# HIITMetagenomics/dsm-framework

Hardware: AMD Instinct MI355X
Metric: enumerated substrings/sec (Emax=2.0) (higher is better)
Workload: dtype u32

## Files before the change

dsm-framework_amd/csrc/emit_runs.h:

```cpp
#pragma once
#include <algorithm>
#include <cstdint>
#include <cstring>
#include <vector>

namespace dsm {

inline void kept_runs(const uint8_t* keep, uint32_t nt, uint8_t drop, std::vector<uint32_t>& seg) {
    seg.clear();
    uint32_t from = 0;
    for (const uint8_t* q = keep; (q = (const uint8_t*)memchr(q, drop, (size_t)(keep + nt - q))) != nullptr; ++q) {
        const uint32_t r = (uint32_t)(q - keep);
        if (r > from) { seg.push_back(from); seg.push_back(r); }
        from = r + 1;
    }
    if (nt > from) { seg.push_back(from); seg.push_back(nt); }
}

inline void rebase_runs(uint32_t* rel_path, uint32_t* rel_pair, const std::vector<uint32_t>& seg, const std::vector<uint32_t>& bp,
                        const std::vector<uint32_t>& bq, uint32_t lo, uint32_t hi) {
    const size_t ns = seg.size() / 2;
    size_t i = (size_t)(std::upper_bound(seg.begin(), seg.end(), lo) - seg.begin()) / 2;
    if (i > 0 && lo <= seg[2 * (i - 1) + 1]) --i;
    for (; i < ns && seg[2 * i] < hi; ++i) {
        const uint32_t a = seg[2 * i] > lo ? seg[2 * i] : lo, b = seg[2 * i + 1] + 1 < hi ? seg[2 * i + 1] + 1 : hi;
        const uint32_t sp = bp[i], sq = bq[i];
        if (!sp && !sq) continue;
        for (uint32_t r = a; r < b; ++r) { rel_path[r] -= sp; rel_pair[r] -= sq; }
    }
}

}
```

dsm-framework_amd/csrc/engine.hip:

```cpp
#include <sched.h>

#include <algorithm>
#include <atomic>
#include <chrono>
#include <cmath>
#include <condition_variable>
#include <cstdlib>
#include <cstring>
#include <deque>
#include <map>
#include <functional>
#include <memory>
#include <mutex>
#include <sstream>
#include <thread>
#include <type_traits>

#include "common.h"
#include "scan.h"
#include "setorder.h"
#include "stream_parse.h"
#include "lfstep.h"
#include "entropy_tables.h"
#include "textemit.h"
#include "engine_api.h"
#include "emit_runs.h"

namespace dsm {

__device__ __forceinline__ u64 wave_sum_u64(u64 v) {
#pragma unroll
    for (int d = 32; d >= 1; d >>= 1) v += __shfl_xor(v, d, 64);
    return v;
}


struct Kids {
    const u64* plane;
    const u32* cum;
};
__device__ __forceinline__ u32 kid_mask(const Kids& k, u32 v) {
    const u64* p = k.plane + (size_t)(v >> 6) * 4;
    const u32 s = v & 63;
    return (u32)((p[0] >> s) & 1) | ((u32)((p[1] >> s) & 1) << 1) | ((u32)((p[2] >> s) & 1) << 2) | ((u32)((p[3] >> s) & 1) << 3);
}
__device__ __forceinline__ u32 kid_index(const Kids& k, u32 v, u32 c) {
    const size_t e = (size_t)(v >> 6) * 4 + c;
    return k.cum[e] + (u32)__popcll(k.plane[e] & ((1ull << (v & 63)) - 1));
}
// ... 1 lines not shown
struct KidWave {
    u64 p[4];
    u32 c[4];
};
__device__ __forceinline__ void kid_wave(const Kids& k, u32 w, KidWave& o) {
#pragma unroll
    for (int c = 0; c < 4; ++c) { o.p[c] = k.plane[(size_t)w * 4 + c]; o.c[c] = k.cum[(size_t)w * 4 + c]; }
}
__device__ __forceinline__ u32 bits_below_lane(u64 p) {
    return __builtin_amdgcn_mbcnt_hi((u32)(p >> 32), __builtin_amdgcn_mbcnt_lo((u32)p, 0u));
}

constexpr u32 NUM_XCD = 8;
__device__ __forceinline__ u32 xcd_block() {
    const u32 b = blockIdx.x, G = gridDim.x;
    const u32 x = b % NUM_XCD, i = b / NUM_XCD, per = G / NUM_XCD, rem = G % NUM_XCD;
    return x * per + (x < rem ? x : rem) + i;
}

constexpr int NPT = 4;
static inline dim3 grid_npt(u64 n) { return dim3((unsigned)((n + 256ull * NPT - 1) / (256ull * NPT))); }


static inline void timeline(const char* what, const char* arg = "") {
    static const bool on = getenv("DSM_TIMELINE") != nullptr;
    if (!on) return;
    static const auto t0 = std::chrono::steady_clock::now();
    fprintf(stderr, "dsm timeline %9.3f ms  %s %s\n", std::chrono::duration<double, std::milli>(std::chrono::steady_clock::now() - t0).count(), what, arg);
}

constexpr u32 BC_OK = 0x4f4b4f4bu, BC_CAPACITY = 0x46554c4cu, BC_ABORT = 0x41424f52u;
constexpr u32 XHDR = 16;
struct ExpandChain {
    struct Link { hipEvent_t last = nullptr; const void* owner = nullptr; };
    std::mutex mu;
    std::map<int, Link> dev;
};
static ExpandChain g_expand_chain;

struct Xchg {
    const u8* base;
    u64 bpr;
    u32 nlocal;
    u32 d;
    u64 F;
    u32 fb;
    u32 nm;
};
__device__ __forceinline__ u64 x_word_index(const Xchg& x, u32 l, u64 v) { return x.nm ? v * x.nlocal + l : (u64)l * x.F + v; }
// ... 918 lines not shown
    u32 r = start[v] + sub[v] - 1;
    slot[r] = RankSlot{k, level};
    if (npair) npair[r] = crec ? 1u : (k + 1 < ncand ? cand_poff[k + 1] : npairs) - cand_poff[k];
}

struct LevelDev {
    const uint2* pw;
    const u32* cand_node;
    const u32* cand_poff;
    const uint4* crec;
    const u32* ids;
    const u64* freqs;
};

constexpr int EMIT_MAX_CHUNKS = 8;
struct ChunkBounds { u32 tb[EMIT_MAX_CHUNKS + 1]; int n; };
__global__ void chunk_bounds_kernel(ChunkBounds cbs, const u32* __restrict__ path_off, const u32* __restrict__ pair_off, u32* __restrict__ out) {
    const int c = threadIdx.x;
    if (c <= cbs.n) { out[2 * c] = path_off[cbs.tb[c]]; out[2 * c + 1] = pair_off ? pair_off[cbs.tb[c]] : cbs.tb[c]; }
}

constexpr u8 EV_DROP = 0, EV_KEEP = 1, EV_HOST = 2;
struct FillVerdict {
    double* ent;
    u8* keep;
    u32* rel_path;
    u32* rel_pair;
    u32* counts;
    const double* terms;
    const double* logn;
    const u32* bounds;
    u32 chunk, d;
    double emin, emax;
};
__global__ __launch_bounds__(256) void tuple_fill_kernel(u32 nlev, const LevelDev* __restrict__ lv, const u32* __restrict__ path_off,
                                                         const u32* __restrict__ pair_off, const RankSlot* __restrict__ slot, char* __restrict__ paths,
                                                         u32* __restrict__ ids, u64* __restrict__ freqs, u32 rank_lo, u32 rank_hi, FillVerdict fv) {
    constexpr u32 LDS_LEVELS = 1024;
    __shared__ const uint2* s_pw[LDS_LEVELS];
    __shared__ u32 s_text[256];
    const u32 nl = nlev < LDS_LEVELS ? nlev : LDS_LEVELS;
    for (u32 q = threadIdx.x; q < nl; q += blockDim.x) s_pw[q] = lv[q].pw;
    {
        const u32 b = threadIdx.x;
        s_text[b] = ((0x54474341u >> (8 * (b & 3))) & 0xFFu) | (((0x54474341u >> (8 * ((b >> 2) & 3))) & 0xFFu) << 8) |
                    (((0x54474341u >> (8 * ((b >> 4) & 3))) & 0xFFu) << 16) | (((0x54474341u >> (8 * ((b >> 6) & 3))) & 0xFFu) << 24);
    }
    __syncthreads();
    const u32 r = rank_lo + blockIdx.x * blockDim.x + threadIdx.x;
    if (r >= rank_hi) return;
    const u32 p_first = path_off[r], p_end = path_off[r + 1];
    const u32 o_first = pair_off ? pair_off[r] : r, o_end = pair_off ? pair_off[r + 1] : r + 1;
    const u32 lvl = p_end - p_first;
    const u32 k = slot[r].k;
    const LevelDev L = lv[lvl];
    const bool one = L.crec != nullptr;
    const uint4 cr = one ? L.crec[k] : make_uint4(0u, 0u, 0u, 0u);
    const u32 b = one ? k : L.cand_poff[k];
    u64 sumN = fv.d;
    double sl = 0;
    bool beyond = false;
    for (u32 q = b, o = o_first; o < o_end; ++q, ++o) {
        const u64 fq = one ? (((u64)cr.w << 32) | cr.z) : L.freqs[q];
        if (ids) ids[o] = one ? 0u : L.ids[q];
        freqs[o] = fq;
        sumN += fq;
        if (fv.ent && !beyond) {
            if (fq < TERM_TAB) sl += fv.terms[fq]; else beyond = true;
        }
    }
    if (fv.ent) {
        beyond = beyond || sumN >= LOGN_TAB;
        u8 verdict = EV_HOST;
        if (!beyond) {
            const double en = fv.logn[sumN] - sl / (double)sumN;
            fv.ent[r] = en;
            verdict = (fv.emax > 0 && (en < fv.emin || en > fv.emax)) ? EV_DROP : EV_KEEP;
        }
        const u32 pb0 = fv.bounds[2 * fv.chunk], qb0 = fv.bounds[2 * fv.chunk + 1];
        fv.keep[r] = verdict;
        fv.rel_path[r + fv.chunk] = p_first - pb0;
        fv.rel_pair[r + fv.chunk] = o_first - qb0;
        if (r + 1 == rank_hi) {
            fv.rel_path[r + 1 + fv.chunk] = p_end - pb0;
            fv.rel_pair[r + 1 + fv.chunk] = o_end - qb0;
        }
        const u64 md = __ballot(verdict == EV_DROP), mh = __ballot(verdict == EV_HOST);
        if ((md | mh) && (threadIdx.x & 63) == (u32)(__ffsll((long long)__ballot(1)) - 1)) {
            if (md) atomicAdd(fv.counts, (u32)__popcll(md));
            if (mh) atomicAdd(fv.counts + 1, (u32)__popcll(mh));
        }
    }
    u32 v = one ? cr.x : L.cand_node[k];
    char* dst = paths + p_first;
    u32 l = lvl;
    while (l > 0) {
        const u32 first = ((l - 1) / PW_CHUNK) * PW_CHUNK;
        const uint2 w = (l < LDS_LEVELS ? s_pw[l] : lv[l].pw)[v];
        const u32 cnt = l - first;
        const u32 q0 = s_text[w.y & 0xFFu], q1 = s_text[(w.y >> 8) & 0xFFu], q2 = s_text[(w.y >> 16) & 0xFFu], q3 = s_text[w.y >> 24];
        char* d = dst + first;
        if (cnt == PW_CHUNK) {
            __builtin_memcpy(d, &q0, 4); __builtin_memcpy(d + 4, &q1, 4); __builtin_memcpy(d + 8, &q2, 4); __builtin_memcpy(d + 12, &q3, 4);
        } else {
            const u32 full = cnt >> 2;
            if (full > 0) __builtin_memcpy(d, &q0, 4);
            if (full > 1) __builtin_memcpy(d + 4, &q1, 4);
            if (full > 2) __builtin_memcpy(d + 8, &q2, 4);
// ... 264 lines not shown
        if (e != hipSuccess) return fail(DSM_E_NOMEM, std::string("hipHostMalloc: ") + hipGetErrorString(e));
        cap = want;
        return 0;
    }
    ~PinBuf() { if (p) (void)hipHostFree(p); }
};
struct DevGrow {
    void* p = nullptr;
    size_t cap = 0;
    int ensure(size_t n) {
        if (n <= cap) return 0;
        if (p) (void)hipFree(p);
        p = nullptr;
        cap = 0;
        size_t want = n + n / 4 + 4096;
        hipError_t e = hipMalloc(&p, want);
        if (e != hipSuccess) return fail(DSM_E_NOMEM, std::string("hipMalloc: ") + hipGetErrorString(e));
        cap = want;
        return 0;
    }
    ~DevGrow() { if (p) (void)hipFree(p); }
};
struct EmitSet {
    DevGrow dev[10];
    hipEvent_t ready = nullptr;
    static constexpr int MAX_CHUNKS = EMIT_MAX_CHUNKS;
    int nchunk = 1;
    u32 cb[MAX_CHUNKS + 1] = {0};
    hipEvent_t cready[MAX_CHUNKS] = {nullptr};
    int device = 0;
    PinBuf pin[10];
    u64 pb[MAX_CHUNKS + 1] = {0}, qb[MAX_CHUNKS + 1] = {0};
    RawBuf out[6];
    u32 nt = 0;
    bool busy = false;
    ~EmitSet() {
        if (ready) (void)hipEventDestroy(ready);
        for (auto e : cready) if (e) (void)hipEventDestroy(e);
    }
};

struct HostPool {
    std::vector<std::thread> th;
    std::mutex mu;
    std::condition_variable cv, done_cv;
    std::function<void(unsigned)> job;
    unsigned gen = 0, pending = 0;
    bool stop = false;
    void ensure(unsigned n) {
        while (th.size() + 1 < n) {
            const unsigned id = (unsigned)th.size() + 1;
            th.emplace_back([this, id] {
                unsigned seen = 0;
                for (;;) {
// ... 18 lines not shown
    unsigned active = 0;
    void run(unsigned n, const std::function<void(unsigned)>& f) {
        ensure(n);
        {
            std::lock_guard<std::mutex> lk(mu);
            job = f; active = n; pending = n - 1; ++gen;
        }
        cv.notify_all();
        f(0u);
        std::unique_lock<std::mutex> lk(mu);
        done_cv.wait(lk, [&] { return pending == 0; });
    }
    ~HostPool() {
        {
            std::lock_guard<std::mutex> lk(mu);
            stop = true;
        }
        cv.notify_all();
        for (auto& t : th) t.join();
    }
};

static int emit_job(HostPool& pool, EmitSet& E, int c, u32 d, double emin, double emax, dsm_tuple_sink sink, void* ctx, std::vector<u32>& zero_ids,
                    u64* n_tuples, u64* n_pairs, double* ms) {
    struct timespec t0, t1;
    clock_gettime(CLOCK_MONOTONIC, &t0);
    const u32 t_lo = E.cb[c], t_hi = E.cb[c + 1];
    const u32 nt = t_hi - t_lo;
    u32* rel_path = (u32*)E.pin[0].p + t_lo + c;
    u32* rel_pair = (u32*)E.pin[1].p + t_lo + c;
    u32* ids = (u32*)E.pin[2].p + E.qb[c];
    if (d == 1) {
        const size_t need = (size_t)rel_pair[nt] + 1;
        if (zero_ids.size() < need) zero_ids.resize(need + need / 4, 0u);
        ids = zero_ids.data();
    }
    u64* freqs = (u64*)E.pin[3].p + E.qb[c];
    char* paths = (char*)E.pin[4].p + E.pb[c];
    double* ent = (double*)E.pin[5].p + t_lo;
    u8* keep = (u8*)E.pin[6].p + t_lo;
    const u32* counts = (const u32*)E.pin[9].p + 2 * c;
    u64 ndrop = counts[0];
    if (counts[1]) {
        for (u8* q = keep; (q = (u8*)memchr(q, EV_HOST, (size_t)(keep + nt - q))) != nullptr; ++q) {
            const u32 r = (u32)(q - keep);
            const double e = exact_entropy(d, freqs + rel_pair[r], rel_pair[r + 1] - rel_pair[r]);
            ent[r] = e;
            const bool k = !(emax > 0 && (e < emin || e > emax));
            keep[r] = k ? EV_KEEP : EV_DROP;
            if (!k) ++ndrop;
        }
    }
    static const bool tl_on = getenv("DSM_TIMELINE") != nullptr;
    if (tl_on) { char msg[96]; snprintf(msg, sizeof msg, "nt=%u dropped=%llu host=%u", nt, (unsigned long long)ndrop, counts[1]); timeline("  emitter: verdicts", msg); }
    u64 W = nt, QW = rel_pair[nt];
    u32* o_path = rel_path;
    u32* o_pair = rel_pair;
    double* o_ent = ent;
    char* o_paths = paths;
    u32* o_ids = ids;
    u64* o_freqs = freqs;
    constexpr u64 FEW_DROPS = 4096;
    if (ndrop && ndrop <= FEW_DROPS && ndrop * 64 < nt) {
        std::vector<u32> seg;
        kept_runs(keep, nt, EV_DROP, seg);
        const size_t ns = seg.size() / 2;
        std::vector<u32> bp(ns), bq(ns);
        for (size_t i = 0; i < ns; ++i) { bp[i] = rel_path[seg[2 * i]]; bq[i] = rel_pair[seg[2 * i]]; }
        unsigned nth = host_threads();
        if (nt < 65536) nth = 1;
        const u32 per = (nt + nth - 1) / nth;
        auto rebase = [&](unsigned t) {
            const u32 lo = t * per < nt ? t * per : nt, hi = t + 1 == nth ? nt + 1 : (lo + per < nt ? lo + per : nt);
            rebase_runs(rel_path, rel_pair, seg, bp, bq, lo, hi);
        };
        pool.run(nth, rebase);
        clock_gettime(CLOCK_MONOTONIC, &t1);
        *ms += (t1.tv_sec - t0.tv_sec) * 1e3 + (t1.tv_nsec - t0.tv_nsec) * 1e-6;
        for (size_t i = 0; i < ns; ++i) {
            const u32 a = seg[2 * i], n = seg[2 * i + 1] - a;
            *n_tuples += n;
            *n_pairs += rel_pair[a + n];
            if (!sink) continue;
            dsm_tuple_batch bt;
            bt.ntuples = n;
            bt.path_off = rel_path + a; bt.path_bytes = paths + bp[i]; bt.entropy = ent + a;
            bt.pair_off = rel_pair + a; bt.ids = ids + bq[i]; bt.freqs = freqs + bq[i];
            if (sink(ctx, &bt)) return 1;
        }
        return 0;
    }
    if (ndrop) {
        unsigned nth = host_threads();
        if (nt < 65536) nth = 1;
        const u32 per = (nt + nth - 1) / nth;
        std::vector<u64> cnt_t(nth + 1, 0), cnt_p(nth + 1, 0), cnt_q(nth + 1, 0);
        auto range = [&](unsigned t, u32& lo, u32& hi) { lo = t * per < nt ? t * per : nt; hi = lo + per < nt ? lo + per : nt; };
        auto pass1 = [&](unsigned t) {
            u32 lo, hi;
            range(t, lo, hi);
            u64 kt = 0, kp = 0, kq = 0;
            for (u32 r = lo; r < hi; ++r)
                if (keep[r] == EV_KEEP) { ++kt; kp += rel_path[r + 1] - rel_path[r]; kq += rel_pair[r + 1] - rel_pair[r]; }
            cnt_t[t + 1] = kt; cnt_p[t + 1] = kp; cnt_q[t + 1] = kq;
        };
        pool.run(nth, pass1);
        for (unsigned t = 0; t < nth; ++t) { cnt_t[t + 1] += cnt_t[t]; cnt_p[t + 1] += cnt_p[t]; cnt_q[t + 1] += cnt_q[t]; }
        W = cnt_t[nth]; QW = cnt_q[nth];
        const u64 PW = cnt_p[nth];
        o_path = (u32*)E.out[0].ensure((W + 1) * 4);
// ... 151 lines not shown
        for (int k = 0; k < 2; ++k) {
            if (buf[k]) (void)hipFree(buf[k]);
            if (ready[k]) (void)hipEventDestroy(ready[k]);
            for (auto e : sev[k]) if (e) (void)hipEventDestroy(e);
        }
        if (copy_stream) (void)hipStreamDestroy(copy_stream);
    }
};

struct Emitter {
    EmitSet set[2];
    HostPool pool;
    std::thread th;
    std::mutex mu;
    std::condition_variable cv;
    std::deque<int> q;
    bool stop = false, started = false;
    int sink_err = 0;
    u32 d = 1;
    double emin = 0, emax = 0;
    dsm_tuple_sink sink = nullptr;
    void* ctx = nullptr;
    std::vector<u32> zero_ids;
    dsm_text_sink text_sink = nullptr;
    TextEmit* te = nullptr;
    std::string text_err;
    u64 tuples = 0, pairs = 0;
    double ms = 0;
    int next = 0;

    int text_job(EmitSet& E, u32 t0, u32 t1, u64* n_tuples, u64* n_pairs, double* ms_) {
        struct timespec a, b;
        clock_gettime(CLOCK_MONOTONIC, &a);
        if (!te) te = text_emit_create(E.device);
        if (!te) return 1;
        const char* text = nullptr;
        size_t len = 0;
        const u32* ids = d == 1 ? nullptr : (const u32*)E.dev[2].p;
        int rc = text_emit_chunk(te, t0, t1, (const u32*)E.dev[0].p, (const u32*)E.dev[1].p, ids, (const u64*)E.dev[3].p, (const char*)E.dev[4].p, d,
                                 emin, emax, &text, &len, n_tuples, n_pairs);
        clock_gettime(CLOCK_MONOTONIC, &b);
        *ms_ += (b.tv_sec - a.tv_sec) * 1e3 + (b.tv_nsec - a.tv_nsec) * 1e-6;
        if (rc) { text_err = dsm_last_error(); return 2; }
        if (len && text_sink(ctx, text, len)) return 1;
        return 0;
    }

    void loop() {
        for (;;) {
            int k;
            {
                std::unique_lock<std::mutex> lk(mu);
                cv.wait(lk, [&] { return stop || !q.empty(); });
                if (q.empty()) return;
                k = q.front();
                q.pop_front();
            }
            u64 t = 0, pq = 0;
            double m = 0;
            (void)hipSetDevice(set[k].device);
            int rc = 0;
            for (int c = 0; c < set[k].nchunk && !rc; ++c) {
                rc = set[k].cready[c] && hipEventSynchronize(set[k].cready[c]) != hipSuccess ? 1 : 0;
                timeline("  emitter: chunk landed");
                if (!rc && set[k].cb[c + 1] > set[k].cb[c]) {
                    if (text_sink) rc = text_job(set[k], set[k].cb[c], set[k].cb[c + 1], &t, &pq, &m);
                    else rc = emit_job(pool, set[k], c, d, emin, emax, sink, ctx, zero_ids, &t, &pq, &m);
                }
                timeline("  emitter: chunk through the sink");
            }
            {
                std::lock_guard<std::mutex> lk(mu);
                tuples += t; pairs += pq; ms += m;
                if (rc) sink_err = rc;
                set[k].busy = false;
            }
            cv.notify_all();
        }
    }
    EmitSet& acquire() {
        std::unique_lock<std::mutex> lk(mu);
        int k = next;
        cv.wait(lk, [&] { return !set[k].busy; });
        return set[k];
    }
    void submit() {
        {
            std::lock_guard<std::mutex> lk(mu);
            if (!started) { started = true; th = std::thread([this] { loop(); }); }
            set[next].busy = true;
// ... 107 lines not shown
    hipEvent_t ev0 = nullptr, ev1 = nullptr;
    std::vector<hipEvent_t> evpool;
    dsm_stats stats;
    u32 splits = 0;
    Emitter emitter;
    dsm_text_sink text_sink_ = nullptr;

    ~Engine() {
        for (void* p : owned) (void)hipFree(p);
        if (h_totals) (void)hipHostFree(h_totals);
        if (h_bounds) (void)hipHostFree(h_bounds);
        if (h_childmax) (void)hipHostFree(h_childmax);
        if (ev0) (void)hipEventDestroy(ev0);
        if (ev1) (void)hipEventDestroy(ev1);
        {
            std::lock_guard<std::mutex> lk(g_expand_chain.mu);
            for (auto& kv : g_expand_chain.dev)
                if (kv.second.owner == this) kv.second = ExpandChain::Link();
        }
        for (hipEvent_t e : evpool) (void)hipEventDestroy(e);
        if (copy_stream) (void)hipStreamDestroy(copy_stream);
        if (fill_done) (void)hipEventDestroy(fill_done);
        for (auto e : chunk_filled) if (e) (void)hipEventDestroy(e);
    }

    template <class T> int dalloc(T*& p, size_t n) {
        void* q = nullptr;
        hipError_t e = hipMalloc(&q, (n ? n : 1) * sizeof(T));
        if (e != hipSuccess) return fail(DSM_E_NOMEM, std::string("hipMalloc: ") + hipGetErrorString(e));
        owned.push_back(q);
        owned_bytes += ((n ? n : 1) * sizeof(T) + 4095) & ~(size_t)4095;
        p = (T*)q;
        return 0;
    }

    int init(dsm_index* const* ix, int n, const dsm_params& p, bool stream) {
        device = ix[0]->device;
        u64 nsum = 0, nmax = 0;
        for (int k = 0; k < n; ++k) {
            if (ix[k]->device != device) return fail(DSM_E_INVAL, "all local indexes must live on one device");
            idx.push_back(ix[k]);
            nsum += ix[k]->meta.n;
            nmax = ix[k]->meta.n > nmax ? ix[k]->meta.n : nmax;
        }
        return init_common(n, p, stream, nsum, nmax);
    }
// ... 342 lines not shown
            if (owner_mode) { if (int rc = owner_precheck(w)) return rc; }
            Sweep s;
            LevelHost child;
            if (int rc = advance(w, s)) return rc;
            if (int rc = publish(w, s)) return rc;
            if (int rc = commit(w, s, child)) return rc;
            if (int rc = capture_level(w, s.Fn, child.slot, child.pw)) return rc;
            if (s.filtered) {
                int erc = emit_store(w.L[w.depth], w.F, w.depth, s.x, w.cur(), w.order_mode, s.crec_cap);
                if (erc == DSM_E_CAPACITY && multi) { w.emit_failed = true; w.emitting = false; }
                else if (erc) return erc;
            }
            DSM_HIP(hipGetLastError());
            if (pend.submit && (w.F >= 200000u || w.depth >= 24)) { if (int rc = flush_pending()) return rc; }
            count_level(w);
            if (!s.Fn) break;
            w.L.push_back(child);
            step(w, s.Fn, s.w16, s.w9);
            if (w.L.size() > 60000) return fail(DSM_E_CAPACITY, "trie deeper than 60000 levels");
        }
        timeline("levels done", w.prefix.c_str());
        if (int rc = flush_pending()) return rc;
        if (int rc = finish_prefix(w, tsink, bsink, ctx)) return rc;
        return read_back(w);
    }

    int root_level(Walk& w) {
        const char* bases = "ACGT";
        for (int s = 0; s < nlocal && trie_mode; ++s) {
            const u32 zero = 0;
            DSM_HIP(hipMemcpyAsync(rp[0][s], &zero, sizeof(u32), hipMemcpyHostToDevice, st));
            stats.reported += tries[s]->nodes;
        }
        for (int s = 0; s < nlocal && !trie_mode; ++s) {
            const IndexMeta& m = idx[s]->meta;
            P h[REC_FIELDS];
            for (int f = 0; f < REC_FIELDS; ++f) h[f] = 0;
            h[0] = 0;
            h[1] = (P)(m.n - 1);
            u8 hmask = 0;
            int slot = 0;
            for (int a = 0; a < 4; ++a) {
                u64 lo = m.C[(int)bases[a]], cnt = m.codes[(int)bases[a]].count;
                if (cnt) { h[2 + 2 * slot] = (P)lo; h[3 + 2 * slot] = (P)(lo + cnt - 1); ++slot; hmask |= (u8)(1u << a); }
            }
            for (int f = 0; f < REC_FIELDS; ++f)
// ... 552 lines not shown
            EARENA_GET(me.ids, u32, me.npairs);
            EARENA_GET(me.freqs, u64, me.npairs);
            me.ncand = nc;
            hipLaunchKernelGGL((cand_store_kernel<P>), grid_npt(F), dim3(256), 0, st, fa, xp, nT[cur], order[cur], order16[cur], me.cand_bits, cand_wscan,
                               me.cand_node, me.cand_poff, me.ids, me.freqs);
        }
        stats.candidates += me.ncand;
        return 0;
    }

    int finish_mine(std::vector<LevelHost>& L, u32 nlev, dsm_tuple_sink sink, void* ctx, bool* ready) {
        u64 ncand_total = 0;
        for (u32 l = 1; l < nlev; ++l) ncand_total += L[l].ncand;
        if (ncand_total == 0) return 0;
        if (ncand_total > 0xFFFFFFF0ull) return fail(DSM_E_CAPACITY, "more than 2^32 candidate tuples in one prefix: use a longer prefix");
        const u32 nt = (u32)ncand_total;
        for (u32 l = nlev; l-- > 1;) {
            EARENA_GET(L[l].sub, u32, L[l].n);
            const u32* child_sub = l + 1 < nlev ? L[l + 1].sub : nullptr;
            hipLaunchKernelGGL((up_bits_kernel<u32>), grid_npt(L[l].n), dim3(256), 0, st, L[l].n, L[l].cand_bits, L[l].kids(), child_sub, L[l].sub);
        }
        const bool text_mode = text_sink_ != nullptr;
        const bool one_pair = d == 1 && !text_mode;
        u32* npair = nullptr;
        if (!one_pair) EARENA_GET(npair, u32, nt);
        u32 maxn = 1;
        for (u32 l = 0; l < nlev; ++l) maxn = L[l].n > maxn ? L[l].n : maxn;
        u32* startbuf[2];
        EARENA_GET(startbuf[0], u32, maxn);
        EARENA_GET(startbuf[1], u32, maxn);
        RankSlot* slot;
        EARENA_GET(slot, RankSlot, nt);
        DSM_HIP(hipMemsetAsync(startbuf[0], 0, sizeof(u32), st));
        for (u32 l = 0; l + 1 < nlev; ++l) {
            u32* s_cur = startbuf[l & 1];
            u32* s_next = startbuf[(l + 1) & 1];
            hipLaunchKernelGGL((down_kernel<u32>), grid_npt(L[l].n), dim3(256), 0, st, L[l].n, s_cur, 0u, L[l].kids(), L[l + 1].sub, s_next);
            if (L[l + 1].ncand)
                hipLaunchKernelGGL(cand_rank_kernel, grid_for(L[l + 1].ncand), dim3(256), 0, st, L[l + 1].ncand, L[l + 1].cand_node, L[l + 1].cand_poff,
                                   L[l + 1].npairs, s_next, L[l + 1].sub, l + 1, slot, npair, L[l + 1].crec);
        }
        std::vector<LevelDev> lv(nlev);
        u64 path_bytes = 0, npairs = 0;
        for (u32 l = 0; l < nlev; ++l) {
            lv[l].pw = L[l].pw; lv[l].cand_node = L[l].cand_node; lv[l].cand_poff = L[l].cand_poff; lv[l].crec = L[l].crec;
            lv[l].ids = L[l].ids; lv[l].freqs = L[l].freqs;
// ... 9 lines not shown
        if (!copy_stream) DSM_HIP(hipStreamCreateWithFlags(&copy_stream, hipStreamNonBlocking));
        if (int rc = E.dev[0].ensure(((size_t)nt + 1) * 4)) return rc;
        if (!one_pair) { if (int rc = E.dev[1].ensure(((size_t)nt + 1) * 4)) return rc; }
        u32* path_off = (u32*)E.dev[0].p;
        u32* pair_off = one_pair ? nullptr : (u32*)E.dev[1].p;
        u32* stmp;
        EARENA_GET(stmp, u32, scan_tmp_elems(nt) + 8);
        exclusive_scan<RankSlot, u32>(slot, path_off, nt, stmp, d_totals, st);
        if (!one_pair) exclusive_scan<u32, u32>(npair, pair_off, nt, stmp, d_totals + 1, st);
        DSM_HIP(hipMemcpyAsync(path_off + nt, d_totals, sizeof(u32), hipMemcpyDeviceToDevice, st));
        if (!one_pair) DSM_HIP(hipMemcpyAsync(pair_off + nt, d_totals + 1, sizeof(u32), hipMemcpyDeviceToDevice, st));
        static const u64 chunk_unit = [] {
            const char* e = getenv("DSM_EMIT_CHUNK_TUPLES");
            const long long n = e ? atoll(e) : 0;
            return n > 0 ? (u64)n : (u64)(1u << 20);
        }();
        ChunkBounds cbs;
        cbs.n = nt >= 4 * chunk_unit ? 4 : (nt >= 2 * chunk_unit ? 2 : 1);
        for (int c = 0; c <= cbs.n; ++c) cbs.tb[c] = (u32)((u64)nt * c / cbs.n);
        u32* d_bounds;
        EARENA_GET(d_bounds, u32, 2 * (EmitSet::MAX_CHUNKS + 1));
        hipLaunchKernelGGL(chunk_bounds_kernel, dim3(1), dim3(64), 0, st, cbs, path_off, pair_off, d_bounds);
        DSM_HIP(hipMemcpyAsync(h_bounds, d_bounds, 2 * (cbs.n + 1) * sizeof(u32), hipMemcpyDeviceToHost, st));
        const bool no_ids = d == 1;
        if (!no_ids) { if (int rc = E.dev[2].ensure((size_t)npairs * 4)) return rc; }
        if (int rc = E.dev[3].ensure((size_t)npairs * 8)) return rc;
        if (int rc = E.dev[4].ensure((size_t)path_bytes)) return rc;
        u32* d_ids = no_ids ? nullptr : (u32*)E.dev[2].p;
        u64* d_freqs = (u64*)E.dev[3].p;
        char* d_paths = (char*)E.dev[4].p;
        emitter.text_sink = text_sink_;
        FillVerdict fv;
        memset(&fv, 0, sizeof fv);
        if (!text_mode) {
            const size_t nrel = (size_t)nt + EmitSet::MAX_CHUNKS + 1;
            if (int rc = E.pin[0].ensure(nrel * 4)) return rc;
            if (int rc = E.pin[1].ensure(nrel * 4)) return rc;
            if (!no_ids) { if (int rc = E.pin[2].ensure((size_t)npairs * 4)) return rc; }
            if (int rc = E.pin[3].ensure((size_t)npairs * 8)) return rc;
            if (int rc = E.pin[4].ensure((size_t)path_bytes)) return rc;
            if (int rc = E.pin[5].ensure((size_t)nt * 8)) return rc;
            if (int rc = E.pin[6].ensure((size_t)nt)) return rc;
            if (int rc = E.pin[9].ensure(2 * EmitSet::MAX_CHUNKS * sizeof(u32))) return rc;
            if (int rc = E.dev[5].ensure((size_t)nt * 8)) return rc;
            if (int rc = E.dev[6].ensure((size_t)nt)) return rc;
            if (int rc = E.dev[7].ensure(nrel * 4)) return rc;
            if (int rc = E.dev[8].ensure(nrel * 4)) return rc;
            if (int rc = E.dev[9].ensure(2 * EmitSet::MAX_CHUNKS * sizeof(u32))) return rc;
            if (!d_terms) {
                if (int rc = dalloc(d_terms, (size_t)TERM_TAB)) return rc;
                if (int rc = dalloc(d_logn, (size_t)LOGN_TAB)) return rc;
                DSM_HIP(hipMemcpyAsync(d_terms, term_table(), (size_t)TERM_TAB * 8, hipMemcpyHostToDevice, st));
                DSM_HIP(hipMemcpyAsync(d_logn, logn_table(), (size_t)LOGN_TAB * 8, hipMemcpyHostToDevice, st));
            }
            DSM_HIP(hipMemsetAsync(E.dev[9].p, 0, 2 * EmitSet::MAX_CHUNKS * sizeof(u32), st));
            fv.ent = (double*)E.dev[5].p; fv.keep = (u8*)E.dev[6].p; fv.rel_path = (u32*)E.dev[7].p; fv.rel_pair = (u32*)E.dev[8].p;
            fv.terms = d_terms; fv.logn = d_logn; fv.d = d; fv.emin = prm.emin; fv.emax = prm.emax; fv.bounds = d_bounds;
        }
        E.nchunk = cbs.n;
        if (!copy_stream) DSM_HIP(hipStreamCreateWithFlags(&copy_stream, hipStreamNonBlocking));
        for (int c = 0; c < cbs.n; ++c) {
            const u32 t0 = cbs.tb[c], t1 = cbs.tb[c + 1];
            fv.chunk = (u32)c;
            fv.counts = text_mode ? nullptr : (u32*)E.dev[9].p + 2 * c;
            if (t1 > t0)
                hipLaunchKernelGGL(tuple_fill_kernel, grid_for(t1 - t0), dim3(256), 0, st, nlev, d_lv, path_off, pair_off, slot, d_paths, d_ids, d_freqs, t0, t1, fv);
            DSM_HIP(hipGetLastError());
            E.cb[c] = t0; E.cb[c + 1] = t1;
            if (!E.cready[c]) DSM_HIP(hipEventCreateWithFlags(&E.cready[c], hipEventDisableTiming));
            if (!chunk_filled[c]) DSM_HIP(hipEventCreateWithFlags(&chunk_filled[c], hipEventDisableTiming));
            DSM_HIP(hipEventRecord(chunk_filled[c], st));
        }
        pend.E = &E; pend.nchunk = cbs.n; pend.text = text_mode; pend.ids = !no_ids;
        E.nt = nt;
        emitter.d = d; emitter.emin = prm.emin; emitter.emax = prm.emax; emitter.sink = sink; emitter.ctx = ctx;
        *ready = true;
        return 0;
    }
    struct PendingEmit {
        EmitSet* E = nullptr;
        int nchunk = 0;
        bool text = false, submit = false, ids = true;
    } pend;
    int flush_pending() {
        if (!pend.E || !pend.submit) return 0;
        EmitSet& E = *pend.E;
        pend.E = nullptr;
        pend.submit = false;
        DSM_HIP(hipSetDevice(device));
        const u32* d_ids = (const u32*)E.dev[2].p;
        const u64* d_freqs = (const u64*)E.dev[3].p;
        const char* d_paths = (const char*)E.dev[4].p;
        for (int c = 0; c < pend.nchunk; ++c) {
            const u32 t0 = E.cb[c], t1 = E.cb[c + 1];
            if (pend.text) {
                DSM_HIP(hipStreamWaitEvent(copy_stream, chunk_filled[c], 0));
                DSM_HIP(hipEventRecord(E.cready[c], copy_stream));
                continue;
            }
            DSM_HIP(hipStreamWaitEvent(copy_stream, chunk_filled[c], 0));
            const u64 pb0 = h_bounds[2 * c], qb0 = h_bounds[2 * c + 1], pb1 = h_bounds[2 * (c + 1)], qb1 = h_bounds[2 * (c + 1) + 1];
            DSM_HIP(hipMemcpyAsync((u32*)E.pin[0].p + t0 + c, (const u32*)E.dev[7].p + t0 + c, ((size_t)(t1 - t0) + 1) * 4, hipMemcpyDeviceToHost, copy_stream));
            DSM_HIP(hipMemcpyAsync((u32*)E.pin[1].p + t0 + c, (const u32*)E.dev[8].p + t0 + c, ((size_t)(t1 - t0) + 1) * 4, hipMemcpyDeviceToHost, copy_stream));
            if (t1 > t0) {
                DSM_HIP(hipMemcpyAsync((double*)E.pin[5].p + t0, (const double*)E.dev[5].p + t0, (size_t)(t1 - t0) * 8, hipMemcpyDeviceToHost, copy_stream));
                DSM_HIP(hipMemcpyAsync((u8*)E.pin[6].p + t0, (const u8*)E.dev[6].p + t0, (size_t)(t1 - t0), hipMemcpyDeviceToHost, copy_stream));
            }
            DSM_HIP(hipMemcpyAsync((u32*)E.pin[9].p + 2 * c, (const u32*)E.dev[9].p + 2 * c, 2 * sizeof(u32), hipMemcpyDeviceToHost, copy_stream));
            E.pb[c] = pb0; E.qb[c] = qb0;
            if (qb1 > qb0) {
                if (pend.ids) DSM_HIP(hipMemcpyAsync((u32*)E.pin[2].p + qb0, d_ids + qb0, (qb1 - qb0) * 4, hipMemcpyDeviceToHost, copy_stream));
                DSM_HIP(hipMemcpyAsync((u64*)E.pin[3].p + qb0, d_freqs + qb0, (qb1 - qb0) * 8, hipMemcpyDeviceToHost, copy_stream));
            }
            if (pb1 > pb0) DSM_HIP(hipMemcpyAsync((char*)E.pin[4].p + pb0, d_paths + pb0, pb1 - pb0, hipMemcpyDeviceToHost, copy_stream));
            DSM_HIP(hipEventRecord(E.cready[c], copy_stream));
        }
        DSM_HIP(hipEventRecord(E.ready, copy_stream));
        emitter.submit();
        return 0;
    }
    hipStream_t copy_stream = nullptr;
    double* d_terms = nullptr;
    double* d_logn = nullptr;
    hipEvent_t fill_done = nullptr;
    hipEvent_t chunk_filled[EmitSet::MAX_CHUNKS] = {nullptr};

    int finish_emits() {
        timeline("finish_emits");
        if (int rc = flush_pending()) return rc;
        timeline("last set submitted");
        emitter.drain();
        timeline("emitter drained");
        std::lock_guard<std::mutex> lk(emitter.mu);
        stats.tuples += emitter.tuples; stats.pairs += emitter.pairs; stats.host_ms += emitter.ms;
        emitter.tuples = emitter.pairs = 0;
        emitter.ms = 0;
        if (emitter.sink_err) {
            const int e = emitter.sink_err;
            emitter.sink_err = 0;
            if (e == 2) return fail(DSM_E_HIP, "text emitter: " + emitter.text_err);
            return fail(DSM_E_SINK, "tuple sink failed");
        }
        return 0;
    }

    int finish_stream(std::vector<LevelHost>& L, u32 nlev, dsm_byte_sink sink, void* ctx) {
        if (nlev < 2) {
            sout.submit(0, 0, stream_tag, 0, 0, stream_last);
// ... 117 lines not shown
}

template <typename P>
struct MinerT : MinerBase {
    Engine<P> e;
    bool stream_mode() const override { return e.stream_mode; }
    int run(const char* prefix, dsm_tuple_sink ts, dsm_byte_sink bs, void* ctx, dsm_stats* out) override {
        const char* one[1] = {prefix};
        return run_many(one, 1, ts, bs, ctx, out);
    }
    int run_auto(const std::string& prefix, dsm_tuple_sink ts, void* ctx, const RunOpts& o) {
        int rc = e.run(prefix.c_str(), ts, nullptr, ctx, o);
        if (rc != DSM_E_CAPACITY || prefix.size() >= 32) return rc;
        ++e.splits;
        if (getenv("DSM_TRACE_SPLITS")) fprintf(stderr, "dsm split rank=%d prefix=%s Fcap=%u: %s\n", e.rank, prefix.c_str(), e.Fcap, dsm_last_error());
        const u32 k = (u32)prefix.size();
        NodeOrder cap;
        cap.depth = k + 1;
        RunOpts shallow = o;
        shallow.emit = false;
        shallow.expand_cap = k + 1;
        shallow.capture = &cap;
        shallow.count = false;
        rc = e.run(prefix.c_str(), ts, nullptr, ctx, shallow);
        if (rc) return rc;
        for (size_t q = 0; q < cap.sym.size(); ++q) {
            NodeOrder sub;
            sub.depth = k + 1;
            sub.ord.push_back(cap.ord[q]);
            RunOpts below = o;
            below.emit_lo = k + 1;
            below.seed = &sub;
            rc = run_auto(prefix + "ACGT"[cap.sym[q]], ts, ctx, below);
            if (rc) return rc;
        }
        RunOpts top = o;
        top.emit_hi = k;
        top.expand_cap = k + 1;
        return e.run(prefix.c_str(), ts, nullptr, ctx, top);
    }
    int stream_auto(const std::string& prefix, void* ctx, u64 rbase, u64 head_skip, u32 tail_levels, bool last, u64* below) {
        const u32 k = (u32)prefix.size();
        e.stream_rbase = rbase; e.stream_head_skip = head_skip; e.stream_tail_levels = tail_levels; e.stream_last = last;
        const u64 before = e.stats.reported;
        int rc = e.run(prefix.c_str(), nullptr, nullptr, ctx);
        if (rc != DSM_E_CAPACITY || k >= 32) {
            const u64 rep = e.stats.reported - before;
            if (below) *below = rep >= k ? rep - k + (k ? 1 : 0) : 0;
            return rc;
        }
        ++e.splits;
        if (getenv("DSM_TRACE_SPLITS")) fprintf(stderr, "dsm split rank=%d prefix=%s Fcap=%u: %s\n", e.rank, prefix.c_str(), e.Fcap, dsm_last_error());
        NodeOrder cap;
        cap.depth = k + 1;
        RunOpts shallow;
// ... 10 lines not shown
                             last && q + 1 == m, &sub);
            if (rc) return rc;
            sum += sub;
        }
        if (m == 0) return fail(DSM_E_CAPACITY, "device arena exhausted: use a larger arena_bytes");
        if (below) *below = sum + (k ? 1 : 0);
        e.stats.reported = before + k + sum;
        return 0;
    }
    int run_many(const char* const* prefixes, int n, dsm_tuple_sink ts, dsm_byte_sink bs, void* ctx, dsm_stats* out,
                 dsm_prefix_byte_sink ps = nullptr, dsm_text_sink xs = nullptr) override {
        memset(&e.stats, 0, sizeof e.stats);
        e.text_sink_ = xs;
        int rc = 0;
        timeline("call begins");
        if (e.stream_mode) { e.sout.sink = bs; e.sout.psink = ps; e.sout.ctx = ctx; }
        for (int k = 0; k < n && !rc; ++k) {
            const bool mine = e.owner_mode ? e.is_owner : (!e.prm.emit_owner_only || e.world <= 1 || (k % e.world) == e.rank);
            e.stream_tag = k;
            if (e.stream_mode) rc = stream_auto(prefixes[k] ? prefixes[k] : "", ctx, 0, 0, 0, true, nullptr);
            else {
                RunOpts o;
                o.emit = mine;
                rc = run_auto(prefixes[k] ? prefixes[k] : "", ts, ctx, o);
            }
        }
        int rc2 = e.finish_emits();
        if (e.stream_mode) {
            const int se = e.sout.drain();
            if (se && !rc2) rc2 = fail(se == 1 ? DSM_E_SINK : DSM_E_HIP, se == 1 ? "byte sink failed" : "copying the wire stream to the host failed");
        }
        e.stats.splits = e.splits;
        e.splits = 0;
        if (out) *out = e.stats;
        return rc ? rc : rc2;
    }
};

template <typename P>
static int mine_impl(dsm_index* const* idx, int n, const dsm_params* p, dsm_tuple_sink sink, void* ctx, dsm_stats* stats) {
    std::unique_ptr<MinerT<P>> m(new MinerT<P>());
    int rc = m->e.init(idx, n, *p, false);
    if (rc) return rc;
    return m->run(p->prefix, sink, nullptr, ctx, stats);
}
template <typename P>
// ... 99 lines not shown
```

dsm-framework_amd/csrc/engine_api.h:

```cpp
#pragma once
#include <string>
#include <vector>

#include "common.h"

struct dsm_trie {
    int device = 0;
    dsm::u64 nodes = 0, maxfreq = 0;
    std::vector<dsm::u64> level_off;
    dsm::u64* d_freq = nullptr;
    dsm::u8* d_pl = nullptr;
    dsm::u32* d_fc = nullptr;
};

namespace dsm {

struct MinerBase {
    virtual ~MinerBase() {}
    virtual bool stream_mode() const = 0;
    virtual int run(const char* prefix, dsm_tuple_sink ts, dsm_byte_sink bs, void* ctx, dsm_stats* out) = 0;
    virtual int run_many(const char* const* prefixes, int n, dsm_tuple_sink ts, dsm_byte_sink bs, void* ctx, dsm_stats* out,
                         dsm_prefix_byte_sink ps = nullptr, dsm_text_sink xs = nullptr) = 0;
};
bool need_wide(dsm_index* const* idx, int n, const dsm_params* p);
MinerBase* miner_create(dsm_index* const* idx, int n, const dsm_params& p, bool stream_mode, int* rc);
int mine_once(dsm_index* const* idx, int n, const dsm_params* p, dsm_tuple_sink sink, void* ctx, dsm_stats* stats);
int enumerate_once(const dsm_index* idx, const char* prefix, u32 fmin, u32 maxdepth, dsm_byte_sink sink, void* ctx, dsm_stats* stats);
int merge_once(bool wide, dsm_trie* const* tr, int n, const dsm_params* p, dsm_tuple_sink sink, void* ctx, dsm_stats* stats);

struct NodeOrder {
    u32 depth = 0;
    std::vector<u32> sym;
    std::vector<std::vector<u16>> ord;
};
struct RunOpts {
    bool emit = true;
    u32 emit_lo = 1, emit_hi = ~0u;
    u32 expand_cap = ~0u;
    const NodeOrder* seed = nullptr;
    NodeOrder* capture = nullptr;
    bool count = true;
};

struct ServerEngines;
ServerEngines* server_engines_create();
void server_engines_destroy(ServerEngines* e);
int server_run(bool wide, dsm_trie* const* tr, int n, const dsm_params& q, const std::string& prefix, dsm_tuple_sink sink, void* ctx,
               const RunOpts& o, dsm_stats* out, ServerEngines* keep = nullptr, int which = 0);

}
```

Before: 19.72 billion.

## Shrink device-to-host emit traffic for single-pair tuples and parallelize host verdicts

When each tuple has exactly one pair (d==1), the emit path no longer copies rel_pair or entropy arrays to the host. It substitutes an iota array for pair offsets and recomputes entropy on the host from the frequencies. When frequencies fit in 32 bits they are staged as u32, halving that copy. Host-side exact-entropy verdicts now run across the thread pool, and on the last prefix the code waits for the bounds copy so the pending flush can happen earlier. These changes add host compute work and more branching in exchange for less PCIe traffic.

```diff
diff --git a/dsm-framework_amd/csrc/emit_fill.h b/dsm-framework_amd/csrc/emit_fill.h
--- /dev/null
+++ b/dsm-framework_amd/csrc/emit_fill.h
@@ -0,0 +1,15 @@
+#pragma once
+#include <cstdint>
+
+namespace dsm {
+
+inline void fill_from_freqs(const uint32_t* staged, uint64_t* freqs, double* ent, const uint8_t* keep, uint8_t host, const double* terms,
+                            const double* logn, uint32_t lo, uint32_t hi) {
+    for (uint32_t r = lo; r < hi; ++r) {
+        const uint64_t f = staged ? (uint64_t)staged[r] : freqs[r];
+        if (staged) freqs[r] = f;
+        if (keep[r] != host) ent[r] = logn[1 + f] - terms[f] / (double)(1 + f);
+    }
+}
+
+}
diff --git a/dsm-framework_amd/csrc/emit_runs.h b/dsm-framework_amd/csrc/emit_runs.h
--- a/dsm-framework_amd/csrc/emit_runs.h
+++ b/dsm-framework_amd/csrc/emit_runs.h
@@ -25,6 +25,10 @@
     for (; i < ns && seg[2 * i] < hi; ++i) {
         const uint32_t a = seg[2 * i] > lo ? seg[2 * i] : lo, b = seg[2 * i + 1] + 1 < hi ? seg[2 * i + 1] + 1 : hi;
         const uint32_t sp = bp[i], sq = bq[i];
+        if (!rel_pair) {
+            if (sp) for (uint32_t r = a; r < b; ++r) rel_path[r] -= sp;
+            continue;
+        }
         if (!sp && !sq) continue;
         for (uint32_t r = a; r < b; ++r) { rel_path[r] -= sp; rel_pair[r] -= sq; }
     }
diff --git a/dsm-framework_amd/csrc/engine.hip b/dsm-framework_amd/csrc/engine.hip
--- a/dsm-framework_amd/csrc/engine.hip
+++ b/dsm-framework_amd/csrc/engine.hip
@@ -25,6 +25,7 @@
 #include "textemit.h"
 #include "engine_api.h"
 #include "emit_runs.h"
+#include "emit_fill.h"
 
 namespace dsm {
 
@@ -72,9 +73,12 @@
 static inline dim3 grid_npt(u64 n) { return dim3((unsigned)((n + 256ull * NPT - 1) / (256ull * NPT))); }
 
 
+static inline bool timeline_on() {
+    static const bool on = getenv("DSM_TIMELINE") != nullptr;
+    return on;
+}
 static inline void timeline(const char* what, const char* arg = "") {
-    static const bool on = getenv("DSM_TIMELINE") != nullptr;
-    if (!on) return;
+    if (!timeline_on()) return;
     static const auto t0 = std::chrono::steady_clock::now();
     fprintf(stderr, "dsm timeline %9.3f ms  %s %s\n", std::chrono::duration<double, std::milli>(std::chrono::steady_clock::now() - t0).count(), what, arg);
 }
@@ -1039,10 +1043,11 @@
 
 constexpr u8 EV_DROP = 0, EV_KEEP = 1, EV_HOST = 2;
 struct FillVerdict {
+    u8* keep;
     double* ent;
-    u8* keep;
     u32* rel_path;
     u32* rel_pair;
+    u32* freq32;
     u32* counts;
     const double* terms;
     const double* logn;
@@ -1080,27 +1085,27 @@
     for (u32 q = b, o = o_first; o < o_end; ++q, ++o) {
         const u64 fq = one ? (((u64)cr.w << 32) | cr.z) : L.freqs[q];
         if (ids) ids[o] = one ? 0u : L.ids[q];
-        freqs[o] = fq;
+        if (fv.freq32) fv.freq32[o] = (u32)fq; else freqs[o] = fq;
         sumN += fq;
-        if (fv.ent && !beyond) {
+        if (fv.keep && !beyond) {
             if (fq < TERM_TAB) sl += fv.terms[fq]; else beyond = true;
         }
     }
-    if (fv.ent) {
+    if (fv.keep) {
         beyond = beyond || sumN >= LOGN_TAB;
         u8 verdict = EV_HOST;
         if (!beyond) {
             const double en = fv.logn[sumN] - sl / (double)sumN;
-            fv.ent[r] = en;
+            if (fv.ent) fv.ent[r] = en;
             verdict = (fv.emax > 0 && (en < fv.emin || en > fv.emax)) ? EV_DROP : EV_KEEP;
         }
         const u32 pb0 = fv.bounds[2 * fv.chunk], qb0 = fv.bounds[2 * fv.chunk + 1];
         fv.keep[r] = verdict;
         fv.rel_path[r + fv.chunk] = p_first - pb0;
-        fv.rel_pair[r + fv.chunk] = o_first - qb0;
+        if (fv.rel_pair) fv.rel_pair[r + fv.chunk] = o_first - qb0;
         if (r + 1 == rank_hi) {
             fv.rel_path[r + 1 + fv.chunk] = p_end - pb0;
-            fv.rel_pair[r + 1 + fv.chunk] = o_end - qb0;
+            if (fv.rel_pair) fv.rel_pair[r + 1 + fv.chunk] = o_end - qb0;
         }
         const u64 md = __ballot(verdict == EV_DROP), mh = __ballot(verdict == EV_HOST);
         if ((md | mh) && (threadIdx.x & 63) == (u32)(__ffsll((long long)__ballot(1)) - 1)) {
@@ -1411,14 +1416,15 @@
     ~DevGrow() { if (p) (void)hipFree(p); }
 };
 struct EmitSet {
-    DevGrow dev[10];
+    DevGrow dev[11];
+    bool one_pair = false, narrow = false;
     hipEvent_t ready = nullptr;
     static constexpr int MAX_CHUNKS = EMIT_MAX_CHUNKS;
     int nchunk = 1;
     u32 cb[MAX_CHUNKS + 1] = {0};
     hipEvent_t cready[MAX_CHUNKS] = {nullptr};
     int device = 0;
-    PinBuf pin[10];
+    PinBuf pin[11];
     u64 pb[MAX_CHUNKS + 1] = {0}, qb[MAX_CHUNKS + 1] = {0};
     RawBuf out[6];
     u32 nt = 0;
@@ -1483,13 +1489,22 @@
 };
 
 static int emit_job(HostPool& pool, EmitSet& E, int c, u32 d, double emin, double emax, dsm_tuple_sink sink, void* ctx, std::vector<u32>& zero_ids,
-                    u64* n_tuples, u64* n_pairs, double* ms) {
+                    std::vector<u32>& iota, u64* n_tuples, u64* n_pairs, double* ms) {
     struct timespec t0, t1;
     clock_gettime(CLOCK_MONOTONIC, &t0);
     const u32 t_lo = E.cb[c], t_hi = E.cb[c + 1];
     const u32 nt = t_hi - t_lo;
+    const bool one_pair = E.one_pair;
     u32* rel_path = (u32*)E.pin[0].p + t_lo + c;
-    u32* rel_pair = (u32*)E.pin[1].p + t_lo + c;
+    u32* rel_pair = one_pair ? nullptr : (u32*)E.pin[1].p + t_lo + c;
+    if (one_pair) {
+        const size_t have = iota.size(), need = (size_t)nt + 1;
+        if (have < need) {
+            iota.resize(need + need / 4);
+            for (size_t q = have; q < iota.size(); ++q) iota[q] = (u32)q;
+        }
+        rel_pair = iota.data();
+    }
     u32* ids = (u32*)E.pin[2].p + E.qb[c];
     if (d == 1) {
         const size_t need = (size_t)rel_pair[nt] + 1;
@@ -1502,15 +1517,43 @@
     u8* keep = (u8*)E.pin[6].p + t_lo;
     const u32* counts = (const u32*)E.pin[9].p + 2 * c;
     u64 ndrop = counts[0];
+    if (one_pair) {
+        const u32* staged = E.narrow ? (const u32*)E.pin[10].p + t_lo : nullptr;
+        const double* terms = term_table();
+        const double* logn = logn_table();
+        unsigned nth = host_threads();
+        if (nt < 65536) nth = 1;
+        const u32 per = (nt + nth - 1) / nth;
+        auto fill = [&](unsigned t) {
+            const u32 lo = t * per < nt ? t * per : nt, hi = lo + per < nt ? lo + per : nt;
+            fill_from_freqs(staged, freqs, ent, keep, EV_HOST, terms, logn, lo, hi);
+        };
+        if (nth > 1) pool.run(nth, fill); else fill(0u);
+    }
     if (counts[1]) {
-        for (u8* q = keep; (q = (u8*)memchr(q, EV_HOST, (size_t)(keep + nt - q))) != nullptr; ++q) {
-            const u32 r = (u32)(q - keep);
-            const double e = exact_entropy(d, freqs + rel_pair[r], rel_pair[r + 1] - rel_pair[r]);
-            ent[r] = e;
-            const bool k = !(emax > 0 && (e < emin || e > emax));
-            keep[r] = k ? EV_KEEP : EV_DROP;
-            if (!k) ++ndrop;
-        }
+        std::vector<u32> hostpos;
+        hostpos.reserve(counts[1]);
+        for (u8* q = keep; (q = (u8*)memchr(q, EV_HOST, (size_t)(keep + nt - q))) != nullptr; ++q) hostpos.push_back((u32)(q - keep));
+        const u32 nh = (u32)hostpos.size();
+        unsigned nth = host_threads();
+        if (nh < 256) nth = 1;
+        const u32 per = (nh + nth - 1) / nth;
+        std::atomic<u64> dropped{0};
+        auto decide = [&](unsigned t) {
+            const u32 lo = t * per < nh ? t * per : nh, hi = lo + per < nh ? lo + per : nh;
+            u64 nd = 0;
+            for (u32 i = lo; i < hi; ++i) {
+                const u32 r = hostpos[i];
+                const double e = exact_entropy(d, freqs + rel_pair[r], rel_pair[r + 1] - rel_pair[r]);
+                ent[r] = e;
+                const bool k = !(emax > 0 && (e < emin || e > emax));
+                keep[r] = k ? EV_KEEP : EV_DROP;
+                if (!k) ++nd;
+            }
+            if (nd) dropped += nd;
+        };
+        if (nth > 1) pool.run(nth, decide); else decide(0u);
+        ndrop += dropped.load();
     }
     static const bool tl_on = getenv("DSM_TIMELINE") != nullptr;
     if (tl_on) { char msg[96]; snprintf(msg, sizeof msg, "nt=%u dropped=%llu host=%u", nt, (unsigned long long)ndrop, counts[1]); timeline("  emitter: verdicts", msg); }
@@ -1533,7 +1576,7 @@
         const u32 per = (nt + nth - 1) / nth;
         auto rebase = [&](unsigned t) {
             const u32 lo = t * per < nt ? t * per : nt, hi = t + 1 == nth ? nt + 1 : (lo + per < nt ? lo + per : nt);
-            rebase_runs(rel_path, rel_pair, seg, bp, bq, lo, hi);
+            rebase_runs(rel_path, one_pair ? nullptr : rel_pair, seg, bp, bq, lo, hi);
         };
         pool.run(nth, rebase);
         clock_gettime(CLOCK_MONOTONIC, &t1);
@@ -1541,12 +1584,12 @@
         for (size_t i = 0; i < ns; ++i) {
             const u32 a = seg[2 * i], n = seg[2 * i + 1] - a;
             *n_tuples += n;
-            *n_pairs += rel_pair[a + n];
+            *n_pairs += one_pair ? n : rel_pair[a + n];
             if (!sink) continue;
             dsm_tuple_batch bt;
             bt.ntuples = n;
             bt.path_off = rel_path + a; bt.path_bytes = paths + bp[i]; bt.entropy = ent + a;
-            bt.pair_off = rel_pair + a; bt.ids = ids + bq[i]; bt.freqs = freqs + bq[i];
+            bt.pair_off = one_pair ? rel_pair : rel_pair + a; bt.ids = ids + bq[i]; bt.freqs = freqs + bq[i];
             if (sink(ctx, &bt)) return 1;
         }
         return 0;
@@ -1744,6 +1787,7 @@
     dsm_tuple_sink sink = nullptr;
     void* ctx = nullptr;
     std::vector<u32> zero_ids;
+    std::vector<u32> iota;
     dsm_text_sink text_sink = nullptr;
     TextEmit* te = nullptr;
     std::string text_err;
@@ -1787,7 +1831,7 @@
                 timeline("  emitter: chunk landed");
                 if (!rc && set[k].cb[c + 1] > set[k].cb[c]) {
                     if (text_sink) rc = text_job(set[k], set[k].cb[c], set[k].cb[c + 1], &t, &pq, &m);
-                    else rc = emit_job(pool, set[k], c, d, emin, emax, sink, ctx, zero_ids, &t, &pq, &m);
+                    else rc = emit_job(pool, set[k], c, d, emin, emax, sink, ctx, zero_ids, iota, &t, &pq, &m);
                 }
                 timeline("  emitter: chunk through the sink");
             }
@@ -1941,6 +1985,7 @@
         if (copy_stream) (void)hipStreamDestroy(copy_stream);
         if (fill_done) (void)hipEventDestroy(fill_done);
         for (auto e : chunk_filled) if (e) (void)hipEventDestroy(e);
+        if (bounds_landed) (void)hipEventDestroy(bounds_landed);
     }
 
     template <class T> int dalloc(T*& p, size_t n) {
@@ -2329,6 +2374,10 @@
         timeline("levels done", w.prefix.c_str());
         if (int rc = flush_pending()) return rc;
         if (int rc = finish_prefix(w, tsink, bsink, ctx)) return rc;
+        if (w.o.last && pend.submit) {
+            DSM_HIP(hipEventSynchronize(bounds_landed));
+            if (int rc = flush_pending()) return rc;
+        }
         return read_back(w);
     }
 
@@ -2927,6 +2976,7 @@
         }
         const bool text_mode = text_sink_ != nullptr;
         const bool one_pair = d == 1 && !text_mode;
+        const bool narrow = one_pair && sizeof(P) == 4 && !trie_mode;
         u32* npair = nullptr;
         if (!one_pair) EARENA_GET(npair, u32, nt);
         u32 maxn = 1;
@@ -2982,12 +3032,14 @@
         EARENA_GET(d_bounds, u32, 2 * (EmitSet::MAX_CHUNKS + 1));
         hipLaunchKernelGGL(chunk_bounds_kernel, dim3(1), dim3(64), 0, st, cbs, path_off, pair_off, d_bounds);
         DSM_HIP(hipMemcpyAsync(h_bounds, d_bounds, 2 * (cbs.n + 1) * sizeof(u32), hipMemcpyDeviceToHost, st));
+        if (!bounds_landed) DSM_HIP(hipEventCreateWithFlags(&bounds_landed, hipEventDisableTiming));
+        DSM_HIP(hipEventRecord(bounds_landed, st));
         const bool no_ids = d == 1;
         if (!no_ids) { if (int rc = E.dev[2].ensure((size_t)npairs * 4)) return rc; }
-        if (int rc = E.dev[3].ensure((size_t)npairs * 8)) return rc;
+        if (!narrow) { if (int rc = E.dev[3].ensure((size_t)npairs * 8)) return rc; }
         if (int rc = E.dev[4].ensure((size_t)path_bytes)) return rc;
         u32* d_ids = no_ids ? nullptr : (u32*)E.dev[2].p;
-        u64* d_freqs = (u64*)E.dev[3].p;
+        u64* d_freqs = narrow ? nullptr : (u64*)E.dev[3].p;
         char* d_paths = (char*)E.dev[4].p;
         emitter.text_sink = text_sink_;
         FillVerdict fv;
@@ -2995,17 +3047,21 @@
         if (!text_mode) {
             const size_t nrel = (size_t)nt + EmitSet::MAX_CHUNKS + 1;
             if (int rc = E.pin[0].ensure(nrel * 4)) return rc;
-            if (int rc = E.pin[1].ensure(nrel * 4)) return rc;
+            if (!one_pair) { if (int rc = E.pin[1].ensure(nrel * 4)) return rc; }
             if (!no_ids) { if (int rc = E.pin[2].ensure((size_t)npairs * 4)) return rc; }
             if (int rc = E.pin[3].ensure((size_t)npairs * 8)) return rc;
             if (int rc = E.pin[4].ensure((size_t)path_bytes)) return rc;
             if (int rc = E.pin[5].ensure((size_t)nt * 8)) return rc;
             if (int rc = E.pin[6].ensure((size_t)nt)) return rc;
             if (int rc = E.pin[9].ensure(2 * EmitSet::MAX_CHUNKS * sizeof(u32))) return rc;
-            if (int rc = E.dev[5].ensure((size_t)nt * 8)) return rc;
+            if (!one_pair) { if (int rc = E.dev[5].ensure((size_t)nt * 8)) return rc; }
             if (int rc = E.dev[6].ensure((size_t)nt)) return rc;
             if (int rc = E.dev[7].ensure(nrel * 4)) return rc;
-            if (int rc = E.dev[8].ensure(nrel * 4)) return rc;
+            if (!one_pair) { if (int rc = E.dev[8].ensure(nrel * 4)) return rc; }
+            if (narrow) {
+                if (int rc = E.pin[10].ensure((size_t)nt * 4)) return rc;
+                if (int rc = E.dev[10].ensure((size_t)nt * 4)) return rc;
+            }
             if (int rc = E.dev[9].ensure(2 * EmitSet::MAX_CHUNKS * sizeof(u32))) return rc;
             if (!d_terms) {
                 if (int rc = dalloc(d_terms, (size_t)TERM_TAB)) return rc;
@@ -3014,10 +3070,13 @@
                 DSM_HIP(hipMemcpyAsync(d_logn, logn_table(), (size_t)LOGN_TAB * 8, hipMemcpyHostToDevice, st));
             }
             DSM_HIP(hipMemsetAsync(E.dev[9].p, 0, 2 * EmitSet::MAX_CHUNKS * sizeof(u32), st));
-            fv.ent = (double*)E.dev[5].p; fv.keep = (u8*)E.dev[6].p; fv.rel_path = (u32*)E.dev[7].p; fv.rel_pair = (u32*)E.dev[8].p;
+            fv.keep = (u8*)E.dev[6].p; fv.rel_path = (u32*)E.dev[7].p;
+            if (!one_pair) { fv.ent = (double*)E.dev[5].p; fv.rel_pair = (u32*)E.dev[8].p; }
+            if (narrow) fv.freq32 = (u32*)E.dev[10].p;
             fv.terms = d_terms; fv.logn = d_logn; fv.d = d; fv.emin = prm.emin; fv.emax = prm.emax; fv.bounds = d_bounds;
         }
         E.nchunk = cbs.n;
+        E.one_pair = one_pair; E.narrow = narrow;
         if (!copy_stream) DSM_HIP(hipStreamCreateWithFlags(&copy_stream, hipStreamNonBlocking));
         for (int c = 0; c < cbs.n; ++c) {
             const u32 t0 = cbs.tb[c], t1 = cbs.tb[c + 1];
@@ -3060,20 +3119,31 @@
             }
             DSM_HIP(hipStreamWaitEvent(copy_stream, chunk_filled[c], 0));
             const u64 pb0 = h_bounds[2 * c], qb0 = h_bounds[2 * c + 1], pb1 = h_bounds[2 * (c + 1)], qb1 = h_bounds[2 * (c + 1) + 1];
-            DSM_HIP(hipMemcpyAsync((u32*)E.pin[0].p + t0 + c, (const u32*)E.dev[7].p + t0 + c, ((size_t)(t1 - t0) + 1) * 4, hipMemcpyDeviceToHost, copy_stream));
-            DSM_HIP(hipMemcpyAsync((u32*)E.pin[1].p + t0 + c, (const u32*)E.dev[8].p + t0 + c, ((size_t)(t1 - t0) + 1) * 4, hipMemcpyDeviceToHost, copy_stream));
+            u64 bytes = 0;
+            auto to_host = [&](void* dst, const void* src, size_t n) {
+                bytes += n;
+                return hipMemcpyAsync(dst, src, n, hipMemcpyDeviceToHost, copy_stream);
+            };
+            DSM_HIP(to_host((u32*)E.pin[0].p + t0 + c, (const u32*)E.dev[7].p + t0 + c, ((size_t)(t1 - t0) + 1) * 4));
+            if (!E.one_pair) DSM_HIP(to_host((u32*)E.pin[1].p + t0 + c, (const u32*)E.dev[8].p + t0 + c, ((size_t)(t1 - t0) + 1) * 4));
             if (t1 > t0) {
-                DSM_HIP(hipMemcpyAsync((double*)E.pin[5].p + t0, (const double*)E.dev[5].p + t0, (size_t)(t1 - t0) * 8, hipMemcpyDeviceToHost, copy_stream));
-                DSM_HIP(hipMemcpyAsync((u8*)E.pin[6].p + t0, (const u8*)E.dev[6].p + t0, (size_t)(t1 - t0), hipMemcpyDeviceToHost, copy_stream));
-            }
-            DSM_HIP(hipMemcpyAsync((u32*)E.pin[9].p + 2 * c, (const u32*)E.dev[9].p + 2 * c, 2 * sizeof(u32), hipMemcpyDeviceToHost, copy_stream));
+                if (!E.one_pair) DSM_HIP(to_host((double*)E.pin[5].p + t0, (const double*)E.dev[5].p + t0, (size_t)(t1 - t0) * 8));
+                DSM_HIP(to_host((u8*)E.pin[6].p + t0, (const u8*)E.dev[6].p + t0, (size_t)(t1 - t0)));
+            }
+            DSM_HIP(to_host((u32*)E.pin[9].p + 2 * c, (const u32*)E.dev[9].p + 2 * c, 2 * sizeof(u32)));
             E.pb[c] = pb0; E.qb[c] = qb0;
             if (qb1 > qb0) {
-                if (pend.ids) DSM_HIP(hipMemcpyAsync((u32*)E.pin[2].p + qb0, d_ids + qb0, (qb1 - qb0) * 4, hipMemcpyDeviceToHost, copy_stream));
-                DSM_HIP(hipMemcpyAsync((u64*)E.pin[3].p + qb0, d_freqs + qb0, (qb1 - qb0) * 8, hipMemcpyDeviceToHost, copy_stream));
-            }
-            if (pb1 > pb0) DSM_HIP(hipMemcpyAsync((char*)E.pin[4].p + pb0, d_paths + pb0, pb1 - pb0, hipMemcpyDeviceToHost, copy_stream));
+                if (pend.ids) DSM_HIP(to_host((u32*)E.pin[2].p + qb0, d_ids + qb0, (qb1 - qb0) * 4));
+                if (E.narrow) DSM_HIP(to_host((u32*)E.pin[10].p + qb0, (const u32*)E.dev[10].p + qb0, (qb1 - qb0) * 4));
+                else DSM_HIP(to_host((u64*)E.pin[3].p + qb0, d_freqs + qb0, (qb1 - qb0) * 8));
+            }
+            if (pb1 > pb0) DSM_HIP(to_host((char*)E.pin[4].p + pb0, d_paths + pb0, pb1 - pb0));
             DSM_HIP(hipEventRecord(E.cready[c], copy_stream));
+            if (timeline_on()) {
+                char msg[96];
+                snprintf(msg, sizeof msg, "chunk %d: %u tuples, %llu bytes", c, t1 - t0, (unsigned long long)bytes);
+                timeline("copies queued", msg);
+            }
         }
         DSM_HIP(hipEventRecord(E.ready, copy_stream));
         emitter.submit();
@@ -3084,6 +3154,7 @@
     double* d_logn = nullptr;
     hipEvent_t fill_done = nullptr;
     hipEvent_t chunk_filled[EmitSet::MAX_CHUNKS] = {nullptr};
+    hipEvent_t bounds_landed = nullptr;
 
     int finish_emits() {
         timeline("finish_emits");
@@ -3247,6 +3318,7 @@
         shallow.expand_cap = k + 1;
         shallow.capture = &cap;
         shallow.count = false;
+        shallow.last = false;
         rc = e.run(prefix.c_str(), ts, nullptr, ctx, shallow);
         if (rc) return rc;
         for (size_t q = 0; q < cap.sym.size(); ++q) {
@@ -3256,6 +3328,7 @@
             RunOpts below = o;
             below.emit_lo = k + 1;
             below.seed = &sub;
+            below.last = false;
             rc = run_auto(prefix + "ACGT"[cap.sym[q]], ts, ctx, below);
             if (rc) return rc;
         }
@@ -3312,6 +3385,7 @@
             else {
                 RunOpts o;
                 o.emit = mine;
+                o.last = k + 1 == n;
                 rc = run_auto(prefixes[k] ? prefixes[k] : "", ts, ctx, o);
             }
         }
diff --git a/dsm-framework_amd/csrc/engine_api.h b/dsm-framework_amd/csrc/engine_api.h
--- a/dsm-framework_amd/csrc/engine_api.h
+++ b/dsm-framework_amd/csrc/engine_api.h
@@ -40,6 +40,7 @@
     const NodeOrder* seed = nullptr;
     NodeOrder* capture = nullptr;
     bool count = true;
+    bool last = false;
 };
 
 struct ServerEngines;
```

After: 20.59 billion (median of 6 runs). 1.04x the previous value.
